# mhauskn/dqn-hfo

Measured on AMD Instinct MI355X. Metric: DQN updates/sec, 1v0 HFO, 4x1024 MLP, minibatch 256, higher is better.
Workload: dtype f32

## Files before the change

### dqn-hfo_amd/capi.py

```python
import ctypes as C
import os

from ._build import LIB, build

MAX_HIDDEN = 8
DP_ID_BYTES = 128
DP_PER_LAYER, DP_HALF_GRADS, DP_SHARD_OPT = 1, 2, 4
DP_UNVERIFIED_OK = 256
TUNE_FP16_WGRAD_PER_LAYER = 1
TUNE_SEPARATE_HEAD_SEED = 2
TUNE_BWD_UNSHIFTED = 4
TUNE_SEPARATE_ACTOR_HEAD_BWD = 8
TUNE_SEPARATE_Q_TRAIN = 16
TUNE_SEPARATE_FIRST_LAYER = 32
TUNE_SEPARATE_CRITIC_FIRST_LAYERS = 64
TUNE_LATE_GATHER = 128
PLAN_FORMS = ("fp16", "data_parallel", "bwd_shifted_critic", "bwd_shifted_actor", "head_wgrad_rides_critic", "head_wgrad_rides_actor",
              "q_train_in_dgrad", "head_seed_fused", "dqda_head_bwd", "critic_l0_rides", "first_layers_merged", "early_gather_l0", "dp_tails_ride")
ACTOR, CRITIC, ACTOR_TARGET, CRITIC_TARGET = 0, 1, 2, 3
KIND_W, KIND_M, KIND_V, KIND_G = 0, 1, 2, 3


class Config(C.Structure):
    _fields_ = [
        ("struct_size", C.c_int32), ("minibatch", C.c_int32), ("state_size", C.c_int32),
        ("num_hidden", C.c_int32), ("hidden", C.c_int32 * MAX_HIDDEN),
        ("replay_capacity", C.c_int32), ("soft_update_freq", C.c_int32),
        ("gamma", C.c_double), ("beta", C.c_double), ("tau", C.c_double),
        ("actor_lr", C.c_float), ("critic_lr", C.c_float), ("momentum", C.c_float),
        ("momentum2", C.c_float), ("delta", C.c_float), ("clip_gradients", C.c_float),
        ("device", C.c_int32), ("dp_world", C.c_int32), ("dp_rank", C.c_int32), ("use_graph", C.c_int32),
        ("seed", C.c_uint64), ("stream", C.c_void_p), ("grad_arena", C.c_void_p),
        ("grad_arena_bytes", C.c_size_t), ("precision", C.c_int32), ("loss_scale", C.c_float),
        ("tuning_flags", C.c_int32),
    ]


class UpdatePlan(C.Structure):
    _fields_ = [("struct_size", C.c_int32), ("forms", C.c_int32), ("launches_single", C.c_int32), ("launches_graph_first", C.c_int32),
                ("launches_in_graph", C.c_int32), ("updates_per_graph", C.c_int32), ("collectives", C.c_int32), ("reserved", C.c_int32)]


fp = C.POINTER(C.c_float)
ip = C.POINTER(C.c_int32)
up = C.POINTER(C.c_uint8)
H = C.c_void_p

SIGNATURES = {
    "dqnhip_default_config": (None, [C.POINTER(Config), C.c_int32]),
# ... 104 lines not shown
```

### dqn-hfo_amd/csrc/gemm_common.hip.h

```cpp
#pragma once
#include <hip/hip_runtime.h>
#include <stdint.h>

namespace dqnhip {

typedef float f32x4 __attribute__((ext_vector_type(4)));

enum GemmMode { GEMM_FWD = 0, GEMM_DGRAD = 1, GEMM_WGRAD = 2 };

constexpr float kLeakySlope = 0.01f;

struct GemmProblem {
  const float* P; int ldp;
  const float* Q; int ldq;
  float* C; int ldc;
  int Pdim, Qdim, Kred;
  const float* bias;
  const float* mask; int ldm;
  float* db;
  float* partial;
  int relu;
  const float* seed_w; float* C2;
  const float* dot_w; float* dot_out;
  float* xcopy_dst; int xcopy_col, xcopy_n;
  int mode;
  int tiles_p, tiles_q, tile_base;
};

constexpr int kMaxGroup = 4;
struct GemmBatch {
  GemmProblem prob[kMaxGroup];
  int n;
  int total_tiles;
};

__device__ __forceinline__ float lrelu_fwd(float x) {
  return fmaxf(x, 0.0f) + kLeakySlope * fminf(x, 0.0f);
}
__device__ __forceinline__ float lrelu_mask(float y) {
  return (y > 0.0f ? 1.0f : 0.0f) + kLeakySlope * (y <= 0.0f ? 1.0f : 0.0f);
}

__device__ __forceinline__ float wave_sum64(float v) {
  v += __builtin_bit_cast(float, __builtin_amdgcn_update_dpp(0, __builtin_bit_cast(int, v), 0xB1, 0xF, 0xF, false));
  v += __builtin_bit_cast(float, __builtin_amdgcn_update_dpp(0, __builtin_bit_cast(int, v), 0x4E, 0xF, 0xF, false));
  v += __builtin_bit_cast(float, __builtin_amdgcn_update_dpp(0, __builtin_bit_cast(int, v), 0x141, 0xF, 0xF, false));
  v += __builtin_bit_cast(float, __builtin_amdgcn_update_dpp(0, __builtin_bit_cast(int, v), 0x140, 0xF, 0xF, false));
  v += __builtin_bit_cast(float, __builtin_amdgcn_update_dpp(0, __builtin_bit_cast(int, v), 0x142, 0xA, 0xF, false));
  v += __builtin_bit_cast(float, __builtin_amdgcn_update_dpp(0, __builtin_bit_cast(int, v), 0x143, 0xC, 0xF, false));
  return __builtin_bit_cast(float, __builtin_amdgcn_readlane(__builtin_bit_cast(int, v), 63));
}

constexpr int kFlagTarget = 1;
constexpr int kFlagGradNorm = 2;

struct TailsArgs {
  const float* loss_partial; int n_loss; const double* q_partial; int n_q;
  float inv_batch; float* critic_tail; float* actor_tail; const int* flags;
  int on;
};
__device__ __forceinline__ void tails_block(const TailsArgs& a, float* sdot , double* sq ) {
  const int t = threadIdx.x;
  float dot = 0.0f; double qs = 0.0;
  if (a.critic_tail != nullptr) for (int i = t; i < a.n_loss; i += 256) dot += a.loss_partial[i];
  if (a.actor_tail != nullptr) for (int i = t; i < a.n_q; i += 256) qs += a.q_partial[i];
#pragma unroll
  for (int off = 32; off > 0; off >>= 1) { dot += __shfl_xor(dot, off, 64); qs += __shfl_xor(qs, off, 64); }
  if ((t & 63) == 0) { sdot[t >> 6] = dot; sq[t >> 6] = qs; }
  __syncthreads();
  if (t != 0) return;
  if (a.critic_tail != nullptr) {
    dot = (sdot[0] + sdot[1]) + (sdot[2] + sdot[3]);
    a.critic_tail[0] = dot * a.inv_batch / 2.0f;
    a.critic_tail[1] = 0.f; a.critic_tail[2] = (*a.flags & kFlagTarget) ? 1.0f : 0.f; a.critic_tail[3] = 0.f;
  }
  if (a.actor_tail != nullptr) {
    qs = (sq[0] + sq[1]) + (sq[2] + sq[3]);
    a.actor_tail[0] = 0.f; a.actor_tail[1] = (float)qs; a.actor_tail[2] = 0.f; a.actor_tail[3] = 0.f;
  }
}

}
```

### dqn-hfo_amd/csrc/gemm_direct.hip.h

```cpp
#pragma once
#include <hip/hip_runtime.h>
#include <hip/hip_ext.h>

#include <cstdlib>

#include "gemm_common.hip.h"

namespace dqnhip {


__device__ __forceinline__ void tile_of_problem(const GemmProblem& pr, int b, int& tile_p, int& tile_q) {
  if ((pr.tiles_p & 7) == 0) {
    const int xcd = b & 7, j = b >> 3;
    tile_q = j % pr.tiles_q;
    tile_p = (j / pr.tiles_q) * 8 + xcd;
  } else {
    tile_q = b % pr.tiles_q;
    tile_p = b / pr.tiles_q;
  }
}
__device__ __forceinline__ void tile_of_block(const GemmBatch& batch, int& pi, int& tile_p, int& tile_q) {
  int b = blockIdx.x;
  pi = 0;
#pragma unroll
  for (int i = 1; i < kMaxGroup; ++i)
    if (i < batch.n && b >= batch.prob[i].tile_base) pi = i;
  const GemmProblem& pr = batch.prob[pi];
  tile_of_problem(pr, b - pr.tile_base, tile_p, tile_q);
}

template <int NACC>
__device__ __forceinline__ void park_accumulators(float* smem, const f32x4 (&acc)[NACC], int wave, int lane) {
  f32x4* s = reinterpret_cast<f32x4*>(smem);
#pragma unroll
  for (int e = 0; e < NACC; ++e) s[(wave * NACC + e) * 64 + lane] = acc[e];
}
template <int NACC>
__device__ __forceinline__ f32x4 reduce_accumulator(const float* smem, int e, int lane) {
  const f32x4* s = reinterpret_cast<const f32x4*>(smem);
  const f32x4 a0 = s[(0 * NACC + e) * 64 + lane], a1 = s[(1 * NACC + e) * 64 + lane];
  const f32x4 a2 = s[(2 * NACC + e) * 64 + lane], a3 = s[(3 * NACC + e) * 64 + lane];
  f32x4 r;
  r.x = (a0.x + a1.x) + (a2.x + a3.x); r.y = (a0.y + a1.y) + (a2.y + a3.y);
  r.z = (a0.z + a1.z) + (a2.z + a3.z); r.w = (a0.w + a1.w) + (a2.w + a3.w);
  return r;
}

#define DQN_MFMA(a, b, c) __builtin_amdgcn_mfma_f32_16x16x4f32((a), (b), (c), 0, 0, 0)
#define DQN_PIN() __builtin_amdgcn_sched_barrier(0)

__device__ __forceinline__ void store_head_seed(const GemmProblem& pr, int q, int p, const f32x4& v, const f32x4& sw) {
  f32x4 dz;
  dz.x = (-sw.x) * lrelu_mask(v.x); dz.y = (-sw.y) * lrelu_mask(v.y);
  dz.z = (-sw.z) * lrelu_mask(v.z); dz.w = (-sw.w) * lrelu_mask(v.w);
  *reinterpret_cast<f32x4*>(pr.C2 + (size_t)q * pr.ldc + p) = dz;
}

__device__ __forceinline__ void store_head_dot(const GemmProblem& pr, int q, int p, int lg, const f32x4& v, const f32x4& dw) {
  float d = fmaf(v.x, dw.x, 0.0f); d = fmaf(v.y, dw.y, d); d = fmaf(v.z, dw.z, d); d = fmaf(v.w, dw.w, d);
  d += __shfl_xor(d, 16, 64);
  d += __shfl_xor(d, 32, 64);
  if (lg == 0) pr.dot_out[(size_t)q * (pr.Pdim >> 4) + (p >> 4)] = d;
}

template <int TP, int TQ>
__device__ __forceinline__ void fwd_direct_body(const GemmProblem& pr, int tile_p, int tile_q, float* smem) {
  constexpr int NACC = TP * TQ;
  const int lane = threadIdx.x & 63, wave = threadIdx.x >> 6;
  const int li = lane & 15, lg = lane >> 4;
  const int p0 = tile_p * 16 * TP, q0 = tile_q * 16 * TQ;
  const int Kw = pr.Kred >> 2;
  const int nkb = Kw >> 4;
  const float* pp[TP];
  const float* qp[TQ];
#pragma unroll
  for (int c = 0; c < TP; ++c) pp[c] = pr.P + (size_t)(p0 + c * 16 + li) * pr.ldp + wave * Kw + lg * 4;
#pragma unroll
  for (int a = 0; a < TQ; ++a) qp[a] = pr.Q + (size_t)(q0 + a * 16 + li) * pr.ldq + wave * Kw + lg * 4;

  f32x4 acc[NACC];
#pragma unroll
  for (int e = 0; e < NACC; ++e) acc[e] = f32x4{0.f, 0.f, 0.f, 0.f};
// ... 315 lines not shown
#define DN_COMPUTE(slot)                                                                \
  { _Pragma("unroll") for (int s = 0; s < 4; ++s) acc[0] = DQN_MFMA((float)rp[slot][s], (float)rq[slot][s], acc[0]); }
  const int nkbN = nkb - nkb % NS;
  if (nkbN > 0) {
#pragma unroll
    for (int i = 0; i < NS; ++i) { DN_LOAD(i, i) DQN_PIN(); }
    int kb = 0;
    for (; kb + NS < nkbN; kb += NS) {
#pragma unroll
      for (int i = 0; i < NS; ++i) { DN_COMPUTE(i) DQN_PIN(); DN_LOAD(i, kb + NS + i) DQN_PIN(); }
    }
#pragma unroll
    for (int i = 0; i < NS; ++i) { DN_COMPUTE(i) }
  }
  for (int kb = nkbN; kb < nkb; ++kb) { DN_LOAD(0, kb) DN_COMPUTE(0) }
#undef DN_LOAD
#undef DN_COMPUTE
  park_accumulators<1>(smem, acc, wave, lane);
  __syncthreads();
  f32x4 v = f32x4{0.f, 0.f, 0.f, 0.f};
  if (wave == 0) v = reduce_accumulator<1>(smem, 0, lane);
  return v;
}
__device__ __forceinline__ void dgrad_narrow_body(const GemmProblem& pr, int tile_p, int tile_q, float* smem) {
  const f32x4 v = dgrad_narrow_tile<4>(pr, tile_p, tile_q, smem);
  if ((threadIdx.x >> 6) == 0) {
    const int lane = threadIdx.x & 63, li = lane & 15, lg = lane >> 4;
    const int q = tile_q * 16 + li, p = tile_p * 16 + (lg << 2);
    *reinterpret_cast<f32x4*>(pr.C + (size_t)q * pr.ldc + p) = v;
  }
}

constexpr int kWgradRing = 4;
template <int TPB, int TQB>
__device__ __forceinline__ void wgrad_direct_body(const GemmProblem& pr, int tile_p, int tile_q, float* smem) {
  constexpr int NACC = TPB * 4 * TQB * 4;
  const int lane = threadIdx.x & 63, wave = threadIdx.x >> 6;
  const int li = lane & 15, lg = lane >> 4;
  const int p0 = tile_p * 64 * TPB, q0 = tile_q * 64 * TQB;
  const int Kw = pr.Kred >> 2;
  const int nst = Kw >> 2;
  const float* pp = pr.P + (size_t)(wave * Kw + lg) * pr.ldp + p0 + li * 4;
  const float* qp = pr.Q + (size_t)(wave * Kw + lg) * pr.ldq + q0 + li * 4;
  const size_t ldp = pr.ldp, ldq = pr.ldq;
  const bool want_db = (pr.db != nullptr) && (tile_p == 0);

  f32x4 acc[NACC];
#pragma unroll
  for (int e = 0; e < NACC; ++e) acc[e] = f32x4{0.f, 0.f, 0.f, 0.f};
  f32x4 dbacc[TQB];
#pragma unroll
  for (int d = 0; d < TQB; ++d) dbacc[d] = f32x4{0.f, 0.f, 0.f, 0.f};
  constexpr int NS = kWgradRing;
  f32x4 rp[NS][TPB], rq[NS][TQB];

#define WG_LOAD(slot, st)                                                               \
  {                                                                                     \
    _Pragma("unroll") for (int b = 0; b < TPB; ++b)                                     \
        rp[slot][b] = *reinterpret_cast<const f32x4*>(pp + (size_t)((st) << 2) * ldp + b * 64); \
    _Pragma("unroll") for (int d = 0; d < TQB; ++d)                                     \
        rq[slot][d] = *reinterpret_cast<const f32x4*>(qp + (size_t)((st) << 2) * ldq + d * 64); \
  }
#define WG_COMPUTE(slot)                                                                \
  {                                                                                     \
    _Pragma("unroll") for (int d = 0; d < TQB; ++d) {                                   \
      dbacc[d].x += rq[slot][d].x; dbacc[d].y += rq[slot][d].y;                         \
      dbacc[d].z += rq[slot][d].z; dbacc[d].w += rq[slot][d].w;                         \
      _Pragma("unroll") for (int qc = 0; qc < 4; ++qc)                                  \
      _Pragma("unroll") for (int b = 0; b < TPB; ++b)                                   \
      _Pragma("unroll") for (int pc = 0; pc < 4; ++pc)                                  \
          acc[((d * 4 + qc) * TPB + b) * 4 + pc] = DQN_MFMA(                            \
              rp[slot][b][pc], rq[slot][d][qc], acc[((d * 4 + qc) * TPB + b) * 4 + pc]); \
    }                                                                                   \
  }

  const int nstN = nst - nst % NS;
  if (nstN > 0) {
#pragma unroll
    for (int i = 0; i < NS; ++i) { WG_LOAD(i, i) DQN_PIN(); }
    int st = 0;
    for (; st + NS < nstN; st += NS) {
#pragma unroll
      for (int i = 0; i < NS; ++i) { WG_COMPUTE(i) DQN_PIN(); WG_LOAD(i, st + NS + i) DQN_PIN(); }
    }
#pragma unroll
    for (int i = 0; i < NS; ++i) { WG_COMPUTE(i) }
  }
  {
    const int rem = nst - nstN;
    if (rem > 0) WG_LOAD(0, nstN)
    if (rem > 1) WG_LOAD(1, nstN + 1)
    if (rem > 2) WG_LOAD(2, nstN + 2)
    if (rem > 0) WG_COMPUTE(0)
    if (rem > 1) WG_COMPUTE(1)
    if (rem > 2) WG_COMPUTE(2)
  }
#undef WG_LOAD
#undef WG_COMPUTE

  park_accumulators<NACC>(smem, acc, wave, lane);
  float* sdb = smem + 4 * NACC * 64 * 4;
  if (want_db) {
#pragma unroll
    for (int d = 0; d < TQB; ++d) {
      f32x4 v = dbacc[d];
      v.x += __shfl_xor(v.x, 16, 64); v.y += __shfl_xor(v.y, 16, 64); v.z += __shfl_xor(v.z, 16, 64); v.w += __shfl_xor(v.w, 16, 64);
      v.x += __shfl_xor(v.x, 32, 64); v.y += __shfl_xor(v.y, 32, 64); v.z += __shfl_xor(v.z, 32, 64); v.w += __shfl_xor(v.w, 32, 64);
      if (lg == 0) reinterpret_cast<f32x4*>(sdb)[(wave * TQB + d) * 16 + li] = v;
    }
  }
  __syncthreads();
  float ssq = 0.0f;
#pragma unroll
  for (int g4 = 0; g4 < TQB * 4 * TPB; ++g4) {
    if ((g4 & 3) == wave) {
      const int b = g4 % TPB, dq = g4 / TPB, qc = dq & 3, d = dq >> 2;
      f32x4 r0 = reduce_accumulator<NACC>(smem, g4 * 4 + 0, lane);
      f32x4 r1 = reduce_accumulator<NACC>(smem, g4 * 4 + 1, lane);
      f32x4 r2 = reduce_accumulator<NACC>(smem, g4 * 4 + 2, lane);
      f32x4 r3 = reduce_accumulator<NACC>(smem, g4 * 4 + 3, lane);
      const int n = q0 + d * 64 + (li << 2) + qc;
#pragma unroll
      for (int r = 0; r < 4; ++r) {
        const int p = p0 + b * 64 + (lg << 4) + (r << 2);
        const f32x4 v = f32x4{r0[r], r1[r], r2[r], r3[r]};
        ssq = fmaf(v.x, v.x, ssq); ssq = fmaf(v.y, v.y, ssq); ssq = fmaf(v.z, v.z, ssq); ssq = fmaf(v.w, v.w, ssq);
        *reinterpret_cast<f32x4*>(pr.C + (size_t)n * pr.ldc + p) = v;
      }
// ... 635 lines not shown
  if (tid < NH * CW) {
    const int j = tid / CW, c = tid % CW;
    float v = 0.0f;
#pragma unroll 8
    for (int g = 0; g < RG; ++g) v += s_acc[(g * NH + j) * CW + c];
    r.dW[(size_t)j * r.H + blk * CW + c] = v;
    ssq = v * v;
  } else if (blk == 0 && tid < NH * CW + NH) {
    const int j = tid - NH * CW;
    float v = 0.0f;
    for (int m = 0; m < r.rows; ++m) v += s_dy[m * NH + j];
    r.db[j] = v;
    ssq = v * v;
  }
  ssq = wave_sum64(ssq);
  __syncthreads();
  if ((tid & 63) == 0) s_acc[tid >> 6] = ssq;
  __syncthreads();
  if (tid == 0 && r.partial != nullptr) r.partial[blk] = (s_acc[0] + s_acc[1]) + (s_acc[2] + s_acc[3]);
}
template <int NH>
__global__ __launch_bounds__(256) void gemm_wgrad_narrow_rider(const GemmBatch batch, const HeadWgradRider rider) {
  extern __shared__ __attribute__((aligned(16))) float smem[];
  if ((int)blockIdx.x < rider.blocks) { head_wgrad_rider<NH>(rider, (int)blockIdx.x, smem); return; }
  int pi, tile_p, tile_q;
  const int blk = (int)blockIdx.x - rider.blocks;
  pi = 0;
#pragma unroll
  for (int i = 1; i < kMaxGroup; ++i) if (i < batch.n && blk >= batch.prob[i].tile_base) pi = i;
  tile_of_problem(batch.prob[pi], blk - batch.prob[pi].tile_base, tile_p, tile_q);
  wgrad_narrow_body<1>(batch.prob[pi], tile_p, tile_q, smem);
}

template <int NH>
__global__ __launch_bounds__(256) void gemm_wgrad_tail(const GemmBatch batch, const HeadWgradRider rider, const TailsArgs tails) {
  extern __shared__ __attribute__((aligned(16))) float smem[];
  int blk = (int)blockIdx.x;
  int tile_p, tile_q;
  if (tails.on && blk == (int)gridDim.x - 1) { tails_block(tails, smem, reinterpret_cast<double*>(smem + 8)); return; }
  if (blk < rider.blocks) { head_wgrad_rider<NH>(rider, blk, smem); return; }
  blk -= rider.blocks;
  const GemmProblem& p0 = batch.prob[1];
  const int n0 = p0.tiles_p * p0.tiles_q;
  if (blk < n0) { tile_of_problem(p0, blk, tile_p, tile_q); wgrad_narrow_body<1>(p0, tile_p, tile_q, smem); return; }
  blk -= n0;
  const GemmProblem& p1 = batch.prob[0];
  tile_of_problem(p1, blk, tile_p, tile_q); wgrad_direct_body<1, 1>(p1, tile_p, tile_q, smem);
}


struct LaunchTimer { hipEvent_t start = nullptr, stop = nullptr; };
inline LaunchTimer& launch_timer() { static thread_local LaunchTimer t; return t; }

template <typename K>
inline hipError_t direct_launch(K kernel, GemmBatch& batch, int BP, int BQ, int lds_bytes, hipStream_t stream) {
  int base = 0;
  for (int i = 0; i < batch.n; ++i) {
    GemmProblem& p = batch.prob[i];
    p.tiles_p = p.Pdim / BP;
    p.tiles_q = p.Qdim / BQ;
    p.tile_base = base;
    base += p.tiles_p * p.tiles_q;
  }
  batch.total_tiles = base;
  LaunchTimer& lt = launch_timer();
  if (lt.start) { hipExtLaunchKernelGGL(kernel, dim3(base), dim3(256), lds_bytes, stream, lt.start, lt.stop, 0, batch); lt.start = lt.stop = nullptr; }
  else hipLaunchKernelGGL(kernel, dim3(base), dim3(256), lds_bytes, stream, batch);
  return hipGetLastError();
}

template <int TP, int TQ>
inline hipError_t fwd_direct_launch(GemmBatch& b, hipStream_t s) {
  return direct_launch(gemm_fwd_direct<TP, TQ>, b, 16 * TP, 16 * TQ, 4 * TP * TQ * 64 * 16, s);
}
template <int TP, int TQ, bool PIN, int NSLOT = 2>
constexpr int fwd_lds_bytes() {
  return 4 * 4 * ((NSLOT * (TP + TQ) * 512 > TP * TQ * 256) ? NSLOT * (TP + TQ) * 512 : TP * TQ * 256);
}
template <int TP, int TQ, bool PIN, int NSLOT = 2>
inline hipError_t fwd_lds_launch(GemmBatch& b, hipStream_t s) {
// ... 40 lines not shown
  int base = 0;
  for (int i = 0; i < batch.n; ++i) {
    GemmProblem& p = batch.prob[i];
    p.tiles_p = p.Pdim / 16; p.tiles_q = p.Qdim / 16; p.tile_base = base;
    base += p.tiles_p * p.tiles_q;
  }
  batch.total_tiles = base;
  LaunchTimer& lt = launch_timer();
  if (lt.start) { hipExtLaunchKernelGGL(gemm_dgrad_narrow_qrider<0>, dim3(base + rider.blocks), dim3(256), 4 * 64 * 16, stream, lt.start, lt.stop, 0, batch, rider); lt.start = lt.stop = nullptr; }
  else hipLaunchKernelGGL(gemm_dgrad_narrow_qrider<0>, dim3(base + rider.blocks), dim3(256), 4 * 64 * 16, stream, batch, rider);
  return hipGetLastError();
}
template <int TPB>
inline hipError_t wgrad_narrow_launch(GemmBatch& b, hipStream_t s) {
  return direct_launch(gemm_wgrad_narrow<TPB>, b, 64 * TPB, 16, 4 * TPB * 4 * 64 * 16 + 4 * 16 * 4, s);
}
template <int NH>
inline hipError_t wgrad_narrow_rider_launch(GemmBatch& batch, const HeadWgradRider& rider, hipStream_t stream) {
  int base = 0;
  for (int i = 0; i < batch.n; ++i) {
    GemmProblem& p = batch.prob[i];
    p.tiles_p = p.Pdim / 64; p.tiles_q = p.Qdim / 16; p.tile_base = base;
    base += p.tiles_p * p.tiles_q;
  }
  batch.total_tiles = base;
  const size_t need = (size_t)(rider.rows * NH + 16 * NH * 16) * sizeof(float);
  const size_t lds = need > (size_t)(4 * 4 * 64 * 16 + 4 * 16 * 4) ? need : (size_t)(4 * 4 * 64 * 16 + 4 * 16 * 4);
  if (lds > 64 * 1024) return hipErrorInvalidValue;
  LaunchTimer& lt = launch_timer();
  if (lt.start) { hipExtLaunchKernelGGL((gemm_wgrad_narrow_rider<NH>), dim3(base + rider.blocks), dim3(256), lds, stream, lt.start, lt.stop, 0, batch, rider); lt.start = lt.stop = nullptr; }
  else hipLaunchKernelGGL((gemm_wgrad_narrow_rider<NH>), dim3(base + rider.blocks), dim3(256), lds, stream, batch, rider);
  return hipGetLastError();
}
template <int NH>
inline hipError_t wgrad_tail_launch(GemmBatch& batch, const HeadWgradRider& rider, hipStream_t stream, const TailsArgs* tails_in = nullptr) {
  TailsArgs tails{}; if (tails_in != nullptr) { tails = *tails_in; tails.on = 1; }
  GemmProblem& w1 = batch.prob[0]; GemmProblem& w0 = batch.prob[1];
  w1.tiles_p = w1.Pdim / 64; w1.tiles_q = w1.Qdim / 64; w1.tile_base = 0;
  w0.tiles_p = w0.Pdim / 64; w0.tiles_q = w0.Qdim / 16; w0.tile_base = w1.tiles_p * w1.tiles_q;
  const int grid = w0.tile_base + w0.tiles_p * w0.tiles_q + rider.blocks + (tails.on ? 1 : 0);
  batch.total_tiles = grid;
  const size_t need = rider.blocks ? (size_t)(rider.rows * NH + 16 * NH * 16) * sizeof(float) : 0;
  const size_t lds = std::max(need, (size_t)(4 * 16 * 64 * 16 + 4 * 16 * 16));
  if (lds > 80 * 1024) return hipErrorInvalidValue;
  LaunchTimer& lt = launch_timer();
  if (lt.start) { hipExtLaunchKernelGGL((gemm_wgrad_tail<NH>), dim3(grid), dim3(256), lds, stream, lt.start, lt.stop, 0, batch, rider, tails); lt.start = lt.stop = nullptr; }
  else hipLaunchKernelGGL((gemm_wgrad_tail<NH>), dim3(grid), dim3(256), lds, stream, batch, rider, tails);
  return hipGetLastError();
}
template <bool DLDS>
inline hipError_t bwd_seq_launch(GemmBatch& batch, hipStream_t stream) {
  GemmProblem& d = batch.prob[0]; GemmProblem& w = batch.prob[1];
  d.tiles_p = d.Pdim / 64; d.tiles_q = d.Qdim / 16; d.tile_base = 0;
  w.tiles_p = w.Pdim / 64; w.tiles_q = w.Qdim / 64; w.tile_base = 0;
  const int nd = d.tiles_p * d.tiles_q, nw = w.tiles_p * w.tiles_q;
  const int grid = nd > nw ? nd : nw;
  batch.total_tiles = grid;
  constexpr int lds = 4 * 16 * 64 * 16 + 4 * 16 * 16;
  LaunchTimer& lt = launch_timer();
  if (lt.start) { hipExtLaunchKernelGGL((gemm_bwd_seq<DLDS>), dim3(grid), dim3(256), lds, stream, lt.start, lt.stop, 0, batch); lt.start = lt.stop = nullptr; }
  else hipLaunchKernelGGL((gemm_bwd_seq<DLDS>), dim3(grid), dim3(256), lds, stream, batch);
  return hipGetLastError();
}
template <typename K>
inline hipError_t direct_prepare(K kernel, int lds_bytes) {
  return hipFuncSetAttribute(reinterpret_cast<const void*>(kernel), hipFuncAttributeMaxDynamicSharedMemorySize, lds_bytes);
}

}
```

### dqn-hfo_amd/csrc/hgemm.hip.h

```cpp
#pragma once
#include <hip/hip_runtime.h>
#include <stdint.h>
#include <stdlib.h>
#include <type_traits>

#include "gemm_common.hip.h"

namespace dqnhip {

typedef _Float16 h16;
typedef __attribute__((ext_vector_type(8))) _Float16 h16x8;
typedef __attribute__((ext_vector_type(16))) float hg_f32x16;
typedef __attribute__((ext_vector_type(4))) float hg_f32x4;

struct HGemm {
  const h16* A; int lda;
  const h16* B; int ldb;
  int M, N, K;
  h16* C16; int ldc16;
  h16* CT16; int ldct16;
  float* C32; int ldc32;
  int n_valid32;
  const float* bias;
  int relu;
// ... 19 lines not shown
__device__ __forceinline__ bool hg_tile_2d(int bid, int tiles_m, int tiles_n, int& tm, int& tn) {
  if ((tiles_m & 1) || (tiles_n & 3) || (((tiles_m >> 1) * (tiles_n >> 2)) & 7)) return false;
  const int xcd = bid & 7, j = bid >> 3;
  const int q = ((j >> 3) << 3) + xcd, jj = j & 7, bn = tiles_n >> 2;
  tm = ((q / bn) << 1) + (jj >> 2);
  tn = ((q % bn) << 2) + (jj & 3);
  return true;
}

#ifdef HG_CLOCKPROBE
__device__ unsigned long long hg_clk[2];
#endif

template <int WM, int WN, int TM = 1>
struct HGCfg {
  static constexpr int NW = (WM * WN >= 4) ? WM * WN : 4;
  static constexpr int NT = NW * 64;
  static constexpr int WK = (WM * WN >= 4) ? 1 : 4 / (WM * WN);
  static constexpr int BM = WM * 64 * TM, BN = WN * 64;
  static constexpr int KSTEP = (WK == 1) ? 64 : 128;
#ifndef HG_STAGES
#define HG_STAGES 4
#endif
  static constexpr int STAGE = (WK == 1) ? (BM + BN) * 128 : 32768;
  static constexpr int STAGES = (STAGE > 32768) ? 3 : HG_STAGES;
  static constexpr int LOADS = STAGE / 1024 / NW;
  static constexpr int NSUB = (WK == 1) ? 4 : 2;
  static constexpr int TLD = BN + 4;
  static constexpr int T_BYTES = WK * BM * TLD * 4;
  static constexpr int PIPE_BYTES = STAGES * STAGE;
  static constexpr int LDS_BYTES = PIPE_BYTES > T_BYTES ? PIPE_BYTES : T_BYTES;
};

template <int N> __device__ __forceinline__ void hg_wait_vm() { asm volatile("s_waitcnt vmcnt(%0)" ::"n"(N) : "memory"); }
#define HG_PIN() __builtin_amdgcn_sched_barrier(0)

typedef __attribute__((__vector_size__(4 * sizeof(short)))) short hg_s16x4;
typedef __attribute__((address_space(3))) hg_s16x4* hg_lds_s16x4_ptr;

template <int WM, int WN, int MODE, int TM = 1>
__device__ __forceinline__ void hgemm_body(const HGemm& g, const int bid) {
  using Cfg = HGCfg<WM, WN, TM>;
  constexpr int NW = Cfg::NW, NT = Cfg::NT;
  constexpr int MI = 2 * TM;
  constexpr bool TA = (MODE & 1) != 0, TB = (MODE & 2) != 0;
  static_assert(MODE == 0 || (NW == 4 && TM == 1), "reduction-major operands: 128x128 and 64x64 tiles only");
  static_assert(TM == 1 || Cfg::WK == 1, "tall wave tiles: no in-workgroup split-K");
#ifdef HG_CLOCKPROBE
  const unsigned long long hg_c0 = clock64(), hg_r0 = wall_clock64();
#endif
  constexpr int WK = Cfg::WK, BM = Cfg::BM, BN = Cfg::BN, STAGES = Cfg::STAGES, TLD = Cfg::TLD;
  constexpr int NSUB = Cfg::NSUB, LOADS = Cfg::LOADS, KSTEP = Cfg::KSTEP;
  extern __shared__ __attribute__((aligned(1024))) unsigned char hg_smem[];
  const int tid = threadIdx.x, lane = tid & 63, w = tid >> 6;
  const int wm = (WK == 1) ? (w >> 1) : 0, wn = (WK == 1) ? (w & 1) : 0;
  const int tiles_n = g.N / BN, tiles_m = g.M / BM;
  int tm, tn;
  if (!(TA && TB && hg_tile_2d(bid, tiles_m, tiles_n, tm, tn))) {
    const int T = hg_tile_of_block(bid, tiles_m * tiles_n);
    tm = T / tiles_n; tn = T % tiles_n;
  }
  const int m0 = tm * BM, n0 = tn * BN;
  const int nk = g.K / KSTEP;

  const int r8 = lane >> 3, pc = lane & 7;
  const int wu = __builtin_amdgcn_readfirstlane(w);
  const uint32_t lds0 = (uint32_t)(uintptr_t)(__attribute__((address_space(3))) unsigned char*)hg_smem;
// ... 17 lines not shown
      const int row_w = (WK == 1) ? (wu & 1) * 64 : 0;
      wbase = (from_a ? g.A + (size_t)m0 * g.lda : g.B + (size_t)n0 * g.ldb) + (size_t)row_w * ld +
              ((WK == 1) ? 0 : (wu >> 1) * 64);
      dma_step = KSTEP;
#pragma unroll
      for (int i = 0; i < LOADS; ++i) {
        const int R = (wu * LOADS + i) * 8 + r8;
        const int c = pc ^ ((R >> 1) & 7);
        voff[i] = (uint32_t)(((i * 8 + r8) * ld + c * 8) * 2);
      }
    }
  } else {
    static_assert(APW + BPW == LOADS, "stage pieces");
    wbase = g.A + (size_t)(m0 + wu * APW * 8) * g.lda;
    wbase_b = g.B + (size_t)(n0 + wu * BPW * 8) * g.ldb;
#pragma unroll
    for (int i = 0; i < LOADS; ++i) {
      const bool pa = i < APW;
      const int rl = pa ? i * 8 : (i - APW) * 8;
      const int R = (pa ? wu * APW * 8 : BM + wu * BPW * 8) + rl + r8;
      const int c = pc ^ ((R >> 1) & 7);
      voff[i] = (uint32_t)(((rl + r8) * (pa ? g.lda : g.ldb) + c * 8) * 2);
    }
  }
  auto issue1 = [&](int kt, int i) {
    const h16* base; uint32_t dst;
    if constexpr (NW == 4 && TM == 1) {
      base = wbase + (size_t)kt * dma_step;
      dst = lds0 + (uint32_t)((kt % STAGES) * Cfg::STAGE + (wu * LOADS + i) * 1024);
    } else {
      base = (i < APW ? wbase : wbase_b) + (size_t)kt * KSTEP;
      dst = lds0 + (uint32_t)((kt % STAGES) * Cfg::STAGE + (i < APW ? (wu * APW + i) : (BM / 8 + wu * BPW + (i - APW))) * 1024);
    }
    asm volatile("s_mov_b32 m0, %2\n\ts_nop 0\n\tglobal_load_lds_dwordx4 %0, %1"
                 :: "v"(voff[i]), "s"(base), "s"(dst) : "memory");
  };

  const int l31 = lane & 31, hi = lane >> 5, sw = (l31 >> 1) & 7;
  int offa[NSUB], offb[NSUB];
#pragma unroll
  for (int s = 0; s < NSUB; ++s) {
    if constexpr (WK == 1) {
      const int o = (((2 * s + hi) ^ sw) << 4) + l31 * 128;
      offa[s] = wm * 64 * TM * 128 + o; offb[s] = (BM + wn * 64) * 128 + o;
    } else {
      const int o = (((2 * w + hi) ^ sw) << 4) + l31 * 128;
      offa[s] = s * 16384 + o; offb[s] = s * 16384 + 8192 + o;
    }
  }

  hg_f32x16 acc[MI][2];
#pragma unroll
  for (int i = 0; i < MI; ++i)
#pragma unroll
    for (int j = 0; j < 2; ++j)
#pragma unroll
      for (int e = 0; e < 16; ++e) acc[i][j][e] = 0.f;

  int tro[2][2] = {{0, 0}, {0, 0}};
  if constexpr (TA || TB) {
    const int t16 = lane & 15, j4 = t16 >> 2, q4 = t16 & 3, gq = (lane >> 4) & 1;
#pragma unroll
    for (int r = 0; r < 2; ++r) {
      const int row = ((WK == 1) ? 0 : 16 * w) + hi * 8 + 4 * r + j4;
      const int chunk = gq * 2 + (q4 >> 1);
      const int o = row * 128 + ((chunk ^ (((row >> 1) & 1) << 2)) << 4) + (q4 & 1) * 8;
      tro[r][0] = ((WK == 1) ? wm * 8192 : 0) + o;
      tro[r][1] = ((WK == 1) ? (BM + wn * 64) * 128 : 8192) + o;
// ... 596 lines not shown
```

### dqn-hfo_amd/csrc/learner.hip

```cpp
#include "learner_internal.hip.h"

using namespace dqnhip;
using namespace dqnhip_host;

namespace dqnhip_host {

thread_local std::string g_err;

void layout_init(NetLayout& l, int in_dim, const dqnhip_config& c, bool actor) {
  l.L = c.num_hidden; l.in_dim = in_dim; l.NH = actor ? kNO : 1;
  l.dims[0] = in_dim; l.kp[0] = round_up(in_dim, c.precision == DQNHIP_FP16 ? 128 : 64);
  for (int i = 0; i < l.L; ++i) { l.dims[i + 1] = c.hidden[i]; l.kp[i + 1] = c.hidden[i]; }
  size_t off = 0, dense = 0;
  int part = 0;
  for (int i = 0; i < l.L; ++i) {
    l.w_off[i] = off; off += (size_t)l.dims[i + 1] * l.kp[i];
    l.b_off[i] = off; off += round_up(l.dims[i + 1], 64);
    dense += (size_t)l.dims[i + 1] * l.dims[i] + l.dims[i + 1];
    l.part_off[i] = part; part += (l.kp[i] / 64) * (l.dims[i + 1] / (i == 0 ? 16 : 64));
  }
  const int H = l.dims[l.L];
  l.hw_off = off; off += round_up_z((size_t)l.NH * H, 64);
  l.hb_off = off; off += 64;
  dense += (size_t)l.NH * H + l.NH;
// ... 117 lines not shown
  return H % kRiderCW == 0 && (size_t)(rows * NH + 256 * NH) * sizeof(float) <= (size_t)64 * 1024;
}
inline bool bwd_is_shifted(const H* h, const NetLayout& l, int rows) {
  bool shifted = l.L >= 2 && rows % 16 == 0 && !(h->cfg.tuning_flags & DQNHIP_TUNE_BWD_UNSHIFTED);
  for (int i = 1; i < l.L && shifted; ++i) shifted = !bwd_layer_is_pair(l, i, rows) && l.kp[i] % 64 == 0 && l.dims[i + 1] % 64 == 0;
  return shifted;
}
int tower_backward(H* h, hipStream_t st, const NetLayout& l, int net, float* garena, float* partial,
                   float** act, float** dZ, int rows, bool want_w, bool input_grad, int in_lo = 0, int in_hi = -1,
                   const HeadWgradRider* rider = nullptr, const QHeadRider* qrider = nullptr, DqdaHeadArgs* fuse = nullptr,
                   const HeadTrainArgs* qtrain = nullptr, const float* qtrain_seed = nullptr, const TailsArgs* tails = nullptr) {
  auto dgrad_of = [&](int i) {
    GemmProblem p{};
    p.mode = GEMM_DGRAD;
    p.P = wat(h, net, l.w_off[i]); p.ldp = l.kp[i];
    p.Q = dZ[i + 1]; p.ldq = l.kp[i + 1];
    p.C = dZ[i]; p.ldc = l.kp[i];
    p.Pdim = l.kp[i]; p.Qdim = rows; p.Kred = l.dims[i + 1];
    p.mask = i > 0 ? act[i] : nullptr; p.ldm = l.kp[i];
    return p;
  };
  auto wgrad_of = [&](int i) {
    GemmProblem p{};
    p.mode = GEMM_WGRAD;
    p.P = act[i]; p.ldp = l.kp[i];
    p.Q = dZ[i + 1]; p.ldq = l.kp[i + 1];
    p.C = garena + l.w_off[i]; p.ldc = l.kp[i];
    p.Pdim = l.kp[i]; p.Qdim = l.dims[i + 1]; p.Kred = rows;
    p.db = garena + l.b_off[i];
    p.partial = partial ? partial + l.part_off[i] : nullptr;
    return p;
  };
  auto lds_ok_of = [&](int i) { return l.dims[i + 1] >= 512 && l.dims[i + 1] % 256 == 0; };
  auto layer_slice = [&](int i) { return (i + 1 < l.L ? l.w_off[i + 1] : l.hw_off) - l.w_off[i]; };
  const bool shifted = want_w && !input_grad && bwd_is_shifted(h, l, rows);
  if (qtrain != nullptr && !(shifted && lds_ok_of(l.L - 1))) return fail("internal: k_dgrad_qtrain needs the shifted schedule and an LDS-staged top layer");
  if (shifted) {
    {
      GemmBatch bd{}; bd.n = 1; bd.prob[0] = dgrad_of(l.L - 1);
      ScopedTiming t(h, 1, st);
      if (qtrain != nullptr) { bd.prob[0].Q = qtrain_seed; HIPCHK(dgrad_qtrain_launch(bd, *qtrain, st)); }
      else if (lds_ok_of(l.L - 1)) HIPCHK((dgrad_lds_launch<1, 1>(bd, st))); else HIPCHK((dgrad_direct_launch<1, 1>(bd, st)));
    }
    for (int i = l.L - 2; i >= 1; --i) {
      GemmBatch b{}; b.n = 2; b.prob[0] = dgrad_of(i); b.prob[1] = wgrad_of(i + 1);
      ScopedTiming t(h, 4, st);
      if (lds_ok_of(i)) HIPCHK((bwd_seq_launch<true>(b, st))); else HIPCHK((bwd_seq_launch<false>(b, st)));
      if (h->comm && h->dp_per_layer) RC(dp_reduce_slice(h, st, net, l.w_off[i + 1], layer_slice(i + 1)));
    }
    {
      GemmBatch b{}; b.n = 2; b.prob[0] = wgrad_of(1); b.prob[1] = wgrad_of(0);
      const HeadWgradRider none{};
      ScopedTiming t(h, 2, st);
      if (l.NH == 1) HIPCHK((wgrad_tail_launch<1>(b, rider ? *rider : none, st, tails))); else HIPCHK((wgrad_tail_launch<kNO>(b, rider ? *rider : none, st, tails)));
      if (h->comm && h->dp_per_layer) RC(dp_reduce_slice(h, st, net, l.w_off[0], layer_slice(0) + layer_slice(1)));
    }
    if (qrider) return fail("internal: the q-head rider found no carrier launch");
    return 0;
  }
  if (tails != nullptr) return fail("internal: the tails block rides in the shifted schedule's last launch only");
  for (int i = l.L - 1; i >= 0; --i) {
    GemmBatch bd{}, bw{};
    const bool need_dx = (i > 0 || input_grad);
    if (need_dx) bd.prob[bd.n++] = dgrad_of(i);
    if (want_w) bw.prob[bw.n++] = wgrad_of(i);
    const bool lds_ok = lds_ok_of(i);
    if (need_dx && want_w) {
      GemmBatch b{}; b.n = 2; b.prob[0] = bd.prob[0]; b.prob[1] = bw.prob[0];
      ScopedTiming t(h, 4, st);
      if (bwd_layer_is_pair(l, i, rows)) {
        if (lds_ok) HIPCHK((bwd_pair_direct_launch<1, true>(b, st))); else HIPCHK((bwd_pair_direct_launch<1, false>(b, st)));
      } else if (lds_ok) HIPCHK((bwd_seq_launch<true>(b, st)));
      else HIPCHK((bwd_seq_launch<false>(b, st)));
    } else if (need_dx && i == 0 && fuse != nullptr) {
      GemmProblem p = bd.prob[0];
      p.P += in_lo; p.C = nullptr; p.Pdim = 16; p.mask = nullptr;
      fuse->pr = p;
      const QHeadRider none{};
      ScopedTiming t(h, 1, st);
      HIPCHK(dqda_head_bwd_launch(*fuse, qrider ? *qrider : none, st));
      qrider = nullptr;
    } else if (need_dx && i == 0 && in_hi > in_lo && rows % 16 == 0) {
      GemmProblem& p = bd.prob[0];
      const int c0 = (in_lo / 16) * 16, c1 = std::min(l.kp[0], (in_hi + 15) / 16 * 16);
      p.P += c0; p.C += c0; p.Pdim = c1 - c0;
      if (p.mask) p.mask += c0;
      ScopedTiming t(h, 1, st);
// ... 827 lines not shown
    }
    for (int kind = 0; kind < 2; ++kind)
      for (int i = 0; i <= L; ++i) RC(halloc(&h->dZ16[kind][i], (size_t)B * h->k16[kind][i]));
    HIPCHK(hgemm_prepare_all());
  }
  {
    std::mt19937_64 rng(cfg->seed * 0x9E3779B97F4A7C15ull + 12345);
    std::normal_distribution<float> nd(0.0f, 0.01f);
    for (int net = 0; net < 2; ++net) {
      const NetLayout& l = layout_of(h, net);
      std::vector<float> dense(l.dense, 0.0f), arena;
      size_t d = 0;
      for (int i = 0; i < l.L; ++i) {
        const size_t nw = (size_t)l.dims[i + 1] * l.dims[i];
        for (size_t e = 0; e < nw; ++e) dense[d + e] = nd(rng);
        d += nw + l.dims[i + 1];
      }
      const int Hh = l.dims[l.L];
      if (net == 0) {
        for (size_t e = 0; e < (size_t)kNA * Hh; ++e) dense[d + e] = nd(rng);
        d += (size_t)kNA * Hh + kNA;
        for (size_t e = 0; e < (size_t)kNP * Hh; ++e) dense[d + e] = nd(rng);
      } else {
        for (size_t e = 0; e < (size_t)Hh; ++e) dense[d + e] = nd(rng);
      }
      dense_to_arena(l, dense.data(), arena);
      HIPCHK(hipMemcpyAsync(h->w[net], arena.data(), l.arena * sizeof(float), hipMemcpyHostToDevice, h->stream));
      HIPCHK(hipStreamSynchronize(h->stream));
      HIPCHK(hipMemcpyAsync(h->w[net + 2], h->w[net], l.arena * sizeof(float), hipMemcpyDeviceToDevice, h->stream));
    }
  }
  HIPCHK(direct_prepare(gemm_bwd_seq<true>, 4 * 16 * 64 * 16 + 4 * 16 * 16));
  HIPCHK(direct_prepare(gemm_bwd_seq<false>, 4 * 16 * 64 * 16 + 4 * 16 * 16));
  HIPCHK(direct_prepare(gemm_wgrad_tail<1>, 80 * 1024));
  HIPCHK(direct_prepare(gemm_wgrad_tail<kNO>, 80 * 1024));
  HIPCHK(direct_prepare((gemm_bwd_pair_direct<1, true>), 4 * 16 * 64 * 16 + 4 * 16 * 16));
  HIPCHK(direct_prepare((gemm_bwd_pair_direct<1, false>), 4 * 16 * 64 * 16 + 4 * 16 * 16));
  HIPCHK(direct_prepare(gemm_fwd_lds<4, 2, false>, 4 * 2 * 6 * 512 * 4));
  HIPCHK(direct_prepare(gemm_fwd_lds<4, 2, true>, 4 * 2 * 6 * 512 * 4));
  RC(sync_dirty16(h));
  HIPCHK(hipStreamSynchronize(h->stream));
  return 0;
}

int dqnhip_destroy(dqnhip_handle h) {
  if (!h) return 0;
  if (h->sharers > 0) return fail("dqnhip_destroy: %d learner(s) still share this learner's layers / replay memory; destroy them first", h->sharers);
  if (h->w_owner) h->w_owner->sharers -= 1;
  if (h->ring_owner) h->ring_owner->sharers -= 1;
  if (h->ring_ev) hipEventDestroy(h->ring_ev);
  hipSetDevice(h->cfg.device);
  dp_destroy_impl(h, false);
  hipStreamSynchronize(h->stream);
  for (auto& r : h->recs) { hipEventDestroy(r.a); hipEventDestroy(r.b); }
  for (auto& g : h->graph_exec) if (g) hipGraphExecDestroy(g);
  for (auto& g : h->graph_small) if (g) hipGraphExecDestroy(g);
  for (int i = 0; i < 2; ++i) {
    if (h->pipe_ev[i]) hipEventDestroy(h->pipe_ev[i]);
    if (h->pipe_idx_pinned[i]) hipHostFree(h->pipe_idx_pinned[i]);
    if (h->pipe_stats[i]) hipHostFree(h->pipe_stats[i]);
  }
  for (int i = 0; i < 4; ++i) hipFree(h->w[i]);
  for (int i = 0; i < 2; ++i) { hipFree(h->m[i]); hipFree(h->v[i]); hipFree(h->part[i]); }
  if (h->own_grad) hipFree(h->grad_base);
  hipFree(h->ring.state); hipFree(h->ring.next); hipFree(h->ring.act); hipFree(h->ring.reward);
  hipFree(h->ring.mc); hipFree(h->ring.term); hipFree(h->st); hipFree(h->done_counter);
  hipFree(h->Xa_s2[0]); hipFree(h->Xa_s2[1]); hipFree(h->Xa_n); hipFree(h->Xc_tr); hipFree(h->Xc_pl2[0]); hipFree(h->Xc_pl2[1]); hipFree(h->Xc_nx);
  for (int p = 0; p < 5; ++p) for (int i = 1; i <= h->L; ++i) hipFree(h->act[p][i]);
// ... 444 lines not shown
```

### include/dqnhip.h

```cpp
#ifndef DQNHIP_H_
#define DQNHIP_H_

#include <stddef.h>
#include <stdint.h>

#ifdef __cplusplus
extern "C" {
#endif

#define DQNHIP_ACTION_SIZE 4
#define DQNHIP_ACTION_PARAM_SIZE 6
#define DQNHIP_ACTOR_OUT 10
#define DQNHIP_MAX_HIDDEN 8

enum dqnhip_net {
  DQNHIP_ACTOR = 0,
  DQNHIP_CRITIC = 1,
  DQNHIP_ACTOR_TARGET = 2,
  DQNHIP_CRITIC_TARGET = 3
};

enum dqnhip_param_kind {
  DQNHIP_KIND_W = 0,
  DQNHIP_KIND_M = 1,
// ... 12 lines not shown
  int32_t hidden[DQNHIP_MAX_HIDDEN];
  int32_t replay_capacity;
  int32_t soft_update_freq;
  double gamma;
  double beta;
  double tau;
  float actor_lr;
  float critic_lr;
  float momentum;
  float momentum2;
  float delta;
  float clip_gradients;
  int32_t device;
  int32_t dp_world;
  int32_t dp_rank;
  int32_t use_graph;
  uint64_t seed;
  void* stream;
  void* grad_arena;
  size_t grad_arena_bytes;
  int32_t precision;
  float loss_scale;
  int32_t tuning_flags;
} dqnhip_config;

#define DQNHIP_TUNE_FP16_WGRAD_PER_LAYER 1
#define DQNHIP_TUNE_SEPARATE_HEAD_SEED 2
#define DQNHIP_TUNE_BWD_UNSHIFTED 4
#define DQNHIP_TUNE_SEPARATE_ACTOR_HEAD_BWD 8
#define DQNHIP_TUNE_SEPARATE_Q_TRAIN 16
#define DQNHIP_TUNE_SEPARATE_FIRST_LAYER 32
#define DQNHIP_TUNE_SEPARATE_CRITIC_FIRST_LAYERS 64
#define DQNHIP_TUNE_LATE_GATHER 128

typedef struct dqnhip_learner* dqnhip_handle;

void dqnhip_default_config(dqnhip_config* cfg, int32_t state_size);

size_t dqnhip_grad_arena_bytes(const dqnhip_config* cfg);

const char* dqnhip_last_error(void);

int dqnhip_create(const dqnhip_config* cfg, dqnhip_handle* out);
int dqnhip_destroy(dqnhip_handle h);


int dqnhip_update(dqnhip_handle h, const int32_t* idx_host,
                  float* critic_loss, float* avg_q);

int dqnhip_update_pipelined(dqnhip_handle h, const int32_t* idx_host,
                            float* critic_loss, float* avg_q);

int dqnhip_update_chained(dqnhip_handle h, const int32_t* idx_host, const int32_t* idx_next,
                          float* critic_loss, float* avg_q);

int dqnhip_update_async(dqnhip_handle h, const int32_t* idx_host);

int dqnhip_update_async_n(dqnhip_handle h, int32_t n);

int dqnhip_update_phase(dqnhip_handle h, int32_t phase, const int32_t* idx_host);
int dqnhip_update_abort(dqnhip_handle h);

int dqnhip_apply_update(dqnhip_handle h, int32_t net);
int dqnhip_apply_update_sharded(dqnhip_handle h, int32_t net, int32_t world);

#define DQNHIP_PLAN_FP16 1
// ... 134 lines not shown
```

Before: 3544.

## Stage wgrad tail operands through LDS with async DMA, eight-deep pipeline

The wgrad tail kernel's direct weight-gradient body now issues global_load_lds DMA copies into an eight-slot LDS ring and reads each step back into a two-entry register pair. Before, it kept a four-deep ring of global loads in registers. The deeper pipeline is meant to hide more global-load latency while cutting register pressure. In exchange it uses more LDS per block and adds waitcnt-based synchronisation. The old register ring stays available behind a new tuning flag.

```diff
diff --git a/dqn-hfo_amd/capi.py b/dqn-hfo_amd/capi.py
--- a/dqn-hfo_amd/capi.py
+++ b/dqn-hfo_amd/capi.py
@@ -15,6 +15,7 @@
 TUNE_SEPARATE_FIRST_LAYER = 32
 TUNE_SEPARATE_CRITIC_FIRST_LAYERS = 64
 TUNE_LATE_GATHER = 128
+TUNE_WGRAD_REGISTER_RING = 256
 PLAN_FORMS = ("fp16", "data_parallel", "bwd_shifted_critic", "bwd_shifted_actor", "head_wgrad_rides_critic", "head_wgrad_rides_actor",
               "q_train_in_dgrad", "head_seed_fused", "dqda_head_bwd", "critic_l0_rides", "first_layers_merged", "early_gather_l0", "dp_tails_ride")
 ACTOR, CRITIC, ACTOR_TARGET, CRITIC_TARGET = 0, 1, 2, 3
diff --git a/dqn-hfo_amd/csrc/gemm_common.hip.h b/dqn-hfo_amd/csrc/gemm_common.hip.h
--- a/dqn-hfo_amd/csrc/gemm_common.hip.h
+++ b/dqn-hfo_amd/csrc/gemm_common.hip.h
@@ -51,6 +51,11 @@
   return __builtin_bit_cast(float, __builtin_amdgcn_readlane(__builtin_bit_cast(int, v), 63));
 }
 
+__device__ __forceinline__ void lds_dma_x4(const void* base, uint32_t voff, uint32_t lds) {
+  asm volatile("s_mov_b32 m0, %2\n\ts_nop 0\n\tglobal_load_lds_dwordx4 %0, %1" :: "v"(voff), "s"(base), "s"(lds) : "memory");
+}
+template <int N> __device__ __forceinline__ void wait_vmcnt() { asm volatile("s_waitcnt vmcnt(%0)" ::"n"(N) : "memory"); }
+
 constexpr int kFlagTarget = 1;
 constexpr int kFlagGradNorm = 2;
 
diff --git a/dqn-hfo_amd/csrc/gemm_direct.hip.h b/dqn-hfo_amd/csrc/gemm_direct.hip.h
--- a/dqn-hfo_amd/csrc/gemm_direct.hip.h
+++ b/dqn-hfo_amd/csrc/gemm_direct.hip.h
@@ -3,6 +3,7 @@
 #include <hip/hip_ext.h>
 
 #include <cstdlib>
+#include <type_traits>
 
 #include "gemm_common.hip.h"
 
@@ -48,6 +49,11 @@
 
 #define DQN_MFMA(a, b, c) __builtin_amdgcn_mfma_f32_16x16x4f32((a), (b), (c), 0, 0, 0)
 #define DQN_PIN() __builtin_amdgcn_sched_barrier(0)
+
+template <int I, int N, typename F>
+__device__ __forceinline__ void static_for(F&& f) {
+  if constexpr (I < N) { f(std::integral_constant<int, I>{}); static_for<I + 1, N>(f); }
+}
 
 __device__ __forceinline__ void store_head_seed(const GemmProblem& pr, int q, int p, const f32x4& v, const f32x4& sw) {
   f32x4 dz;
@@ -429,7 +435,12 @@
 }
 
 constexpr int kWgradRing = 4;
-template <int TPB, int TQB>
+template <int TPB, int TQB> constexpr int wgrad_park_bytes() { return 4 * (TPB * 4 * TQB * 4) * 64 * 16 + 4 * TQB * 16 * 16; }
+template <int TPB, int TQB> constexpr int wgrad_low_slots() { return (TPB * 4 * TQB * 4) * 64 * 16 / ((TPB + TQB) * 1024); }
+template <int TPB, int TQB, int SD> constexpr int wgrad_lds_bytes() {
+  return wgrad_park_bytes<TPB, TQB>() + 4 * (SD > wgrad_low_slots<TPB, TQB>() ? SD - wgrad_low_slots<TPB, TQB>() : 0) * (TPB + TQB) * 1024;
+}
+template <int TPB, int TQB, int SD = 0>
 __device__ __forceinline__ void wgrad_direct_body(const GemmProblem& pr, int tile_p, int tile_q, float* smem) {
   constexpr int NACC = TPB * 4 * TQB * 4;
   const int lane = threadIdx.x & 63, wave = threadIdx.x >> 6;
@@ -448,7 +459,7 @@
   f32x4 dbacc[TQB];
 #pragma unroll
   for (int d = 0; d < TQB; ++d) dbacc[d] = f32x4{0.f, 0.f, 0.f, 0.f};
-  constexpr int NS = kWgradRing;
+  constexpr int NS = SD > 0 ? 2 : kWgradRing;
   f32x4 rp[NS][TPB], rq[NS][TQB];
 
 #define WG_LOAD(slot, st)                                                               \
@@ -471,6 +482,73 @@
     }                                                                                   \
   }
 
+  if constexpr (SD > 0) {
+    static_assert(SD % 2 == 0 && SD >= 4, "the register pair alternates inside a block of SD steps");
+    constexpr int NI = TPB + TQB;
+    constexpr int SB = NI * 1024, LOW = wgrad_low_slots<TPB, TQB>(), PARKW = NACC * 64 * 16;
+    const int wu = __builtin_amdgcn_readfirstlane(wave);
+    const uint32_t lds0 = (uint32_t)(uintptr_t)(__attribute__((address_space(3))) unsigned char*)smem;
+    const uint32_t low0 = lds0 + (uint32_t)(wu * PARKW);
+    const uint32_t high0 = lds0 + (uint32_t)(wgrad_park_bytes<TPB, TQB>() + wu * (SD > LOW ? SD - LOW : 0) * SB);
+    auto slot_addr = [&](int slot) { return slot < LOW ? low0 + (uint32_t)(slot * SB) : high0 + (uint32_t)((slot - LOW) * SB); };
+    const float* pw = pr.P + (size_t)(wu * Kw) * pr.ldp + p0;
+    const float* qw = pr.Q + (size_t)(wu * Kw) * pr.ldq + q0;
+    const uint32_t vop = (uint32_t)((lg * pr.ldp + li * 4) * 4), voq = (uint32_t)((lg * pr.ldq + li * 4) * 4);
+    auto issue = [&](int st, int slot) {
+      const uint32_t a = slot_addr(slot);
+#pragma unroll
+      for (int b = 0; b < TPB; ++b) lds_dma_x4(pw + (size_t)(st << 2) * ldp + b * 64, vop, a + b * 1024);
+#pragma unroll
+      for (int d = 0; d < TQB; ++d) lds_dma_x4(qw + (size_t)(st << 2) * ldq + d * 64, voq, a + (TPB + d) * 1024);
+    };
+    typedef __attribute__((address_space(3))) const f32x4* lds_f32x4_ptr;
+#define WG_READ(buf, slot)                                                                            \
+    {                                                                                                 \
+      const uint32_t a = slot_addr(slot) + (uint32_t)(lane * 16);                                     \
+      _Pragma("unroll") for (int b = 0; b < TPB; ++b) rp[buf][b] = *(lds_f32x4_ptr)(uintptr_t)(a + b * 1024);    \
+      _Pragma("unroll") for (int d = 0; d < TQB; ++d) rq[buf][d] = *(lds_f32x4_ptr)(uintptr_t)(a + (TPB + d) * 1024); \
+    }
+    const int nstN = nst - nst % SD;
+    if (nstN > 0) {
+#pragma unroll
+      for (int i = 0; i < SD; ++i) issue(i, i);
+      wait_vmcnt<(SD - 1) * NI>();
+      WG_READ(0, 0)
+      int st = 0;
+      for (; st + SD < nstN; st += SD) {
+#pragma unroll
+        for (int i = 0; i < SD; ++i) {
+          wait_vmcnt<(SD - 2) * NI>();
+          WG_READ((i + 1) & 1, (i + 1) % SD)
+          DQN_PIN();
+          WG_COMPUTE(i & 1)
+          DQN_PIN();
+          issue(st + SD + i, i);
+          DQN_PIN();
+        }
+      }
+      static_for<0, SD>([&](auto ic) {
+        constexpr int i = decltype(ic)::value;
+        if constexpr (i + 1 < SD) {
+          wait_vmcnt<(SD - 2 - i) * NI>();
+          WG_READ((i + 1) & 1, i + 1)
+        }
+        DQN_PIN();
+        WG_COMPUTE(i & 1)
+        DQN_PIN();
+      });
+    }
+    {
+      const int rem = nst - nstN;
+#pragma unroll
+      for (int j = 0; j < SD - 1; ++j) if (j < rem) issue(nstN + j, j);
+      if (rem > 0) wait_vmcnt<0>();
+#pragma unroll
+      for (int j = 0; j < SD - 1; ++j)
+        if (j < rem) { WG_READ(0, j) WG_COMPUTE(0) }
+    }
+#undef WG_READ
+  } else {
   const int nstN = nst - nst % NS;
   if (nstN > 0) {
 #pragma unroll
@@ -491,6 +569,7 @@
     if (rem > 0) WG_COMPUTE(0)
     if (rem > 1) WG_COMPUTE(1)
     if (rem > 2) WG_COMPUTE(2)
+  }
   }
 #undef WG_LOAD
 #undef WG_COMPUTE
@@ -1192,7 +1271,7 @@
   wgrad_narrow_body<1>(batch.prob[pi], tile_p, tile_q, smem);
 }
 
-template <int NH>
+template <int NH, int SD = 0>
 __global__ __launch_bounds__(256) void gemm_wgrad_tail(const GemmBatch batch, const HeadWgradRider rider, const TailsArgs tails) {
   extern __shared__ __attribute__((aligned(16))) float smem[];
   int blk = (int)blockIdx.x;
@@ -1205,7 +1284,7 @@
   if (blk < n0) { tile_of_problem(p0, blk, tile_p, tile_q); wgrad_narrow_body<1>(p0, tile_p, tile_q, smem); return; }
   blk -= n0;
   const GemmProblem& p1 = batch.prob[0];
-  tile_of_problem(p1, blk, tile_p, tile_q); wgrad_direct_body<1, 1>(p1, tile_p, tile_q, smem);
+  tile_of_problem(p1, blk, tile_p, tile_q); wgrad_direct_body<1, 1, SD>(p1, tile_p, tile_q, smem);
 }
 
 
@@ -1312,7 +1391,8 @@
   else hipLaunchKernelGGL((gemm_wgrad_narrow_rider<NH>), dim3(base + rider.blocks), dim3(256), lds, stream, batch, rider);
   return hipGetLastError();
 }
-template <int NH>
+constexpr int kWgradStage = 8;
+template <int NH, int SD = kWgradStage>
 inline hipError_t wgrad_tail_launch(GemmBatch& batch, const HeadWgradRider& rider, hipStream_t stream, const TailsArgs* tails_in = nullptr) {
   TailsArgs tails{}; if (tails_in != nullptr) { tails = *tails_in; tails.on = 1; }
   GemmProblem& w1 = batch.prob[0]; GemmProblem& w0 = batch.prob[1];
@@ -1321,11 +1401,11 @@
   const int grid = w0.tile_base + w0.tiles_p * w0.tiles_q + rider.blocks + (tails.on ? 1 : 0);
   batch.total_tiles = grid;
   const size_t need = rider.blocks ? (size_t)(rider.rows * NH + 16 * NH * 16) * sizeof(float) : 0;
-  const size_t lds = std::max(need, (size_t)(4 * 16 * 64 * 16 + 4 * 16 * 16));
+  const size_t lds = std::max(need, (size_t)wgrad_lds_bytes<1, 1, SD>());
   if (lds > 80 * 1024) return hipErrorInvalidValue;
   LaunchTimer& lt = launch_timer();
-  if (lt.start) { hipExtLaunchKernelGGL((gemm_wgrad_tail<NH>), dim3(grid), dim3(256), lds, stream, lt.start, lt.stop, 0, batch, rider, tails); lt.start = lt.stop = nullptr; }
-  else hipLaunchKernelGGL((gemm_wgrad_tail<NH>), dim3(grid), dim3(256), lds, stream, batch, rider, tails);
+  if (lt.start) { hipExtLaunchKernelGGL((gemm_wgrad_tail<NH, SD>), dim3(grid), dim3(256), lds, stream, lt.start, lt.stop, 0, batch, rider, tails); lt.start = lt.stop = nullptr; }
+  else hipLaunchKernelGGL((gemm_wgrad_tail<NH, SD>), dim3(grid), dim3(256), lds, stream, batch, rider, tails);
   return hipGetLastError();
 }
 template <bool DLDS>
diff --git a/dqn-hfo_amd/csrc/hgemm.hip.h b/dqn-hfo_amd/csrc/hgemm.hip.h
--- a/dqn-hfo_amd/csrc/hgemm.hip.h
+++ b/dqn-hfo_amd/csrc/hgemm.hip.h
@@ -75,7 +75,7 @@
   static constexpr int LDS_BYTES = PIPE_BYTES > T_BYTES ? PIPE_BYTES : T_BYTES;
 };
 
-template <int N> __device__ __forceinline__ void hg_wait_vm() { asm volatile("s_waitcnt vmcnt(%0)" ::"n"(N) : "memory"); }
+template <int N> __device__ __forceinline__ void hg_wait_vm() { wait_vmcnt<N>(); }
 #define HG_PIN() __builtin_amdgcn_sched_barrier(0)
 
 typedef __attribute__((__vector_size__(4 * sizeof(short)))) short hg_s16x4;
@@ -159,8 +159,7 @@
       base = (i < APW ? wbase : wbase_b) + (size_t)kt * KSTEP;
       dst = lds0 + (uint32_t)((kt % STAGES) * Cfg::STAGE + (i < APW ? (wu * APW + i) : (BM / 8 + wu * BPW + (i - APW))) * 1024);
     }
-    asm volatile("s_mov_b32 m0, %2\n\ts_nop 0\n\tglobal_load_lds_dwordx4 %0, %1"
-                 :: "v"(voff[i]), "s"(base), "s"(dst) : "memory");
+    lds_dma_x4(base, voff[i], dst);
   };
 
   const int l31 = lane & 31, hi = lane >> 5, sw = (l31 >> 1) & 7;
diff --git a/dqn-hfo_amd/csrc/learner.hip b/dqn-hfo_amd/csrc/learner.hip
--- a/dqn-hfo_amd/csrc/learner.hip
+++ b/dqn-hfo_amd/csrc/learner.hip
@@ -173,6 +173,7 @@
     return p;
   };
   auto lds_ok_of = [&](int i) { return l.dims[i + 1] >= 512 && l.dims[i + 1] % 256 == 0; };
+  const bool ring = (h->cfg.tuning_flags & DQNHIP_TUNE_WGRAD_REGISTER_RING) != 0;
   auto layer_slice = [&](int i) { return (i + 1 < l.L ? l.w_off[i + 1] : l.hw_off) - l.w_off[i]; };
   const bool shifted = want_w && !input_grad && bwd_is_shifted(h, l, rows);
   if (qtrain != nullptr && !(shifted && lds_ok_of(l.L - 1))) return fail("internal: k_dgrad_qtrain needs the shifted schedule and an LDS-staged top layer");
@@ -193,7 +194,11 @@
       GemmBatch b{}; b.n = 2; b.prob[0] = wgrad_of(1); b.prob[1] = wgrad_of(0);
       const HeadWgradRider none{};
       ScopedTiming t(h, 2, st);
-      if (l.NH == 1) HIPCHK((wgrad_tail_launch<1>(b, rider ? *rider : none, st, tails))); else HIPCHK((wgrad_tail_launch<kNO>(b, rider ? *rider : none, st, tails)));
+      const HeadWgradRider& r = rider ? *rider : none;
+      if (ring) {
+        if (l.NH == 1) HIPCHK((wgrad_tail_launch<1, 0>(b, r, st, tails))); else HIPCHK((wgrad_tail_launch<kNO, 0>(b, r, st, tails)));
+      } else if (l.NH == 1) HIPCHK((wgrad_tail_launch<1>(b, r, st, tails)));
+      else HIPCHK((wgrad_tail_launch<kNO>(b, r, st, tails)));
       if (h->comm && h->dp_per_layer) RC(dp_reduce_slice(h, st, net, l.w_off[0], layer_slice(0) + layer_slice(1)));
     }
     if (qrider) return fail("internal: the q-head rider found no carrier launch");
@@ -1087,8 +1092,10 @@
   }
   HIPCHK(direct_prepare(gemm_bwd_seq<true>, 4 * 16 * 64 * 16 + 4 * 16 * 16));
   HIPCHK(direct_prepare(gemm_bwd_seq<false>, 4 * 16 * 64 * 16 + 4 * 16 * 16));
-  HIPCHK(direct_prepare(gemm_wgrad_tail<1>, 80 * 1024));
-  HIPCHK(direct_prepare(gemm_wgrad_tail<kNO>, 80 * 1024));
+  HIPCHK(direct_prepare(gemm_wgrad_tail<1, 0>, 80 * 1024));
+  HIPCHK(direct_prepare(gemm_wgrad_tail<kNO, 0>, 80 * 1024));
+  HIPCHK(direct_prepare(gemm_wgrad_tail<1, kWgradStage>, 80 * 1024));
+  HIPCHK(direct_prepare(gemm_wgrad_tail<kNO, kWgradStage>, 80 * 1024));
   HIPCHK(direct_prepare((gemm_bwd_pair_direct<1, true>), 4 * 16 * 64 * 16 + 4 * 16 * 16));
   HIPCHK(direct_prepare((gemm_bwd_pair_direct<1, false>), 4 * 16 * 64 * 16 + 4 * 16 * 16));
   HIPCHK(direct_prepare(gemm_fwd_lds<4, 2, false>, 4 * 2 * 6 * 512 * 4));
diff --git a/include/dqnhip.h b/include/dqnhip.h
--- a/include/dqnhip.h
+++ b/include/dqnhip.h
@@ -68,6 +68,7 @@
 #define DQNHIP_TUNE_SEPARATE_FIRST_LAYER 32
 #define DQNHIP_TUNE_SEPARATE_CRITIC_FIRST_LAYERS 64
 #define DQNHIP_TUNE_LATE_GATHER 128
+#define DQNHIP_TUNE_WGRAD_REGISTER_RING 256
 
 typedef struct dqnhip_learner* dqnhip_handle;
 
```

New measurement: 3564 (median of 6 runs). Within noise of the previous version (+0.5%).
